# Enter-tainer/oavif

Measured on AMD Instinct MI355X. Metric: ssimulacra2_megapixels_per_sec, higher is better.
Workload: dtype f32; 1 GPU; ssimulacra2 score of one 3840x2160 RGB8 (ref, dist) pair per step per GPU (BASELINE configs[1]); steps rotate over 16 distinct pairs per GPU = 796 MB of frames resident in HBM (> the 256 MiB Infinity Cache); width=3840, height=2160, distinct_pairs_per_gpu=16, parallelism=single gpu, streams_per_gpu=2

## Files before the change

include/ssimu2_hip_internal.h:

```cpp
#ifndef SSIMU2_HIP_INTERNAL_H_
#define SSIMU2_HIP_INTERNAL_H_

#include "ssimu2_hip.h"

#ifdef __cplusplus
extern "C" {
#endif
#if defined(__GNUC__)
#pragma GCC visibility push(default)
#endif

enum { SSIMU2_DEBUG_LIN_REF = 0, SSIMU2_DEBUG_LIN_DIST = 1, SSIMU2_DEBUG_XYB_REF = 2, SSIMU2_DEBUG_REF_BLUR = 3,
       SSIMU2_DEBUG_RG_H = 4, SSIMU2_DEBUG_RG_V = 5 };
int ssimu2_debug_download(ssimu2_ctx* ctx, int what, int scale, uint32_t w, uint32_t h, float* out,
                          uint32_t* out_w, uint32_t* out_h);

int ssimu2_time_device(ssimu2_ctx* ctx, const void* d_ref, const void* d_dist, uint32_t w,
                       uint32_t h, int iters, float* out_ms_total, double* out_score);

enum { SSIMU2_STAGE_PYRAMID = 0, SSIMU2_STAGE_MARCH = 1, SSIMU2_STAGE_FINALIZE = 2 };
int ssimu2_time_stage(ssimu2_ctx* ctx, const void* d_ref, const void* d_dist, uint32_t w, uint32_t h,
                      int stage, int iters, float* out_ms_avg);

int ssimu2_time_march_rotating(ssimu2_ctx* ctx, const void* const* d_refs, const void* const* d_dists,
                               int npairs, uint32_t w, uint32_t h, int iters, float* out_ms_avg);

int ssimu2_measure_read_stream(ssimu2_ctx* ctx, size_t bytes, int iters, double* out_gbps);

int ssimu2_instr_set_segment_rows(ssimu2_ctx* ctx, int rows_scale0, int rows_other_scales);
int ssimu2_instr_cache_reference_blur(ssimu2_ctx* ctx, int enabled);
int ssimu2_instr_set_batch_segment_rows(ssimu2_ctx* ctx, int rows_scale0);
int ssimu2_instr_batch_segment_rows(ssimu2_ctx* ctx, uint32_t w, uint32_t h, int scale, int* out_rows);
int ssimu2_time_blur_stage_rotating(ssimu2_ctx* ctx, const void* const* d_frames, int nframes, uint32_t w,
                                    uint32_t h, int iters, float* out_ms_avg, double* out_bytes_per_launch);
int ssimu2_time_kernels(ssimu2_ctx* ctx, const void* d_ref, const void* const* d_refs, const void* const* d_dists, int n,
                        uint32_t w, uint32_t h, int iters, float* out_ms_avg, int* out_launches, float* out_ms_wall_timed,
                        float* out_ms_wall_plain);
int ssimu2_instr_placed_streams(ssimu2_ctx* ctx, int* out_n);
int ssimu2_instr_rg_stop_after_scale(ssimu2_ctx* ctx, int scale);

#if defined(__GNUC__)
#pragma GCC visibility pop
#endif
#ifdef __cplusplus
}
#endif
#endif
```

oavif_amd/_lib.py:

```python
from __future__ import annotations

import ctypes
import os

_HERE = os.path.dirname(os.path.abspath(__file__))
LIB_PATH = os.environ.get("OAVIF_AMD_LIB") or os.path.join(_HERE, "lib", "liboavif_hip.so")
INSTR_LIB_PATH = os.environ.get("OAVIF_AMD_INSTR_LIB") or os.path.join(_HERE, "lib", "liboavif_hip_instr.so")

OK = 0
ERR_INVALID_ARG = -1
ERR_UNSUPPORTED = -2
ERR_OOM = -3
ERR_HIP = -4
ERR_NO_REFERENCE = -5
ERR_NO_DEVICE = -6

STAGE_PYRAMID, STAGE_MARCH, STAGE_FINALIZE = 0, 1, 2
NUM_SCALES = 6
STATS_PER_SCALE = 18
TQ_MAX_PASS = 12
MAX_BATCH = 4096

BLUR_FIR, BLUR_RECURSIVE, BLUR_RECURSIVE_FMA = 0, 1, 2

# ... 57 lines not shown

    def __init__(self):
        super().__init__()
        self.struct_size = ctypes.sizeof(DeviceInfo)

    def as_dict(self) -> dict:
        return {"device": int(self.device), "arch": self.arch.decode(), "name": self.name.decode(),
                "pci_bus_id": self.pci_bus_id.decode(), "compute_units": int(self.compute_units),
                "lds_bytes_per_cu": int(self.lds_bytes_per_cu), "lds_bytes_per_workgroup": int(self.lds_bytes_per_workgroup),
                "wavefront_size": int(self.wavefront_size), "hbm_bytes": int(self.hbm_bytes),
                "numa_node": int(self.numa_node), "usable": bool(self.usable)}


class TQSpecStats(ctypes.Structure):
    _fields_ = [("waves", ctypes.c_uint32), ("probes_issued", ctypes.c_uint32),
                ("cache_hits", ctypes.c_uint32)]


INSTR_SYMBOLS = ("ssimu2_debug_download", "ssimu2_time_device", "ssimu2_time_stage",
                 "ssimu2_time_march_rotating", "ssimu2_measure_read_stream",
                 "ssimu2_instr_set_segment_rows", "ssimu2_instr_cache_reference_blur",
                 "ssimu2_instr_rg_stop_after_scale", "ssimu2_time_blur_stage_rotating",
                 "ssimu2_instr_placed_streams", "ssimu2_time_kernels",
                 "ssimu2_instr_set_batch_segment_rows", "ssimu2_instr_batch_segment_rows")

TQ_MAX_FANOUT = 16
BATCH_PROBE_FN = ctypes.CFUNCTYPE(ctypes.c_int, ctypes.c_void_p, ctypes.POINTER(ctypes.c_uint32),
                                  ctypes.c_uint32, ctypes.POINTER(ctypes.c_double))
PROBE_FN = ctypes.CFUNCTYPE(ctypes.c_int, ctypes.c_void_p, ctypes.c_uint32,
                            ctypes.POINTER(ctypes.c_double))
CODEC_FN = ctypes.CFUNCTYPE(ctypes.c_int, ctypes.c_void_p, ctypes.c_uint32,
                            ctypes.POINTER(ctypes.c_uint8), ctypes.POINTER(ctypes.c_size_t))

_lib = None
_instr = None


def lib() -> ctypes.CDLL:
    global _lib
    if _lib is None:
        _lib = _load(LIB_PATH, False)
    return _lib


def instr_lib() -> ctypes.CDLL:
    global _instr
    if _instr is None:
# ... 71 lines not shown
        L.ssimu2_score_rgb16.restype = ci
        L.ssimu2_set_reference_rgb16.argtypes = [vp, u16p, u32, u32, u32]
        L.ssimu2_set_reference_rgb16.restype = ci
        L.ssimu2_score_against_reference_rgb16.argtypes = [vp, u16p, u32, f64p]
        L.ssimu2_score_against_reference_rgb16.restype = ci
        L.ssimu2_score_against_reference_strided16.argtypes = [vp, u16p, u32, u32, u32, f64p]
        L.ssimu2_score_against_reference_strided16.restype = ci
    if hasattr(L, "ssimu2_score_batch_rgb8"):
        u8pp = ctypes.POINTER(u8p)
        L.ssimu2_score_batch_rgb8.argtypes = [vp, u8pp, u8pp, u32, u32, u32, f64p]
        L.ssimu2_score_batch_rgb8.restype = ci
        L.ssimu2_score_batch_against_reference.argtypes = [vp, u8pp, u32, f64p]
        L.ssimu2_score_batch_against_reference.restype = ci
        L.ssimu2_score_batch_rgb8_device.argtypes = [vp, vp, vp, ctypes.c_size_t, u32, u32, u32, f64p]
        L.ssimu2_score_batch_rgb8_device.restype = ci
        L.ssimu2_score_batch_against_reference_device.argtypes = [vp, vp, ctypes.c_size_t, u32, f64p]
        L.ssimu2_score_batch_against_reference_device.restype = ci
        L.ssimu2_last_batch_averages.argtypes = [vp, u32, f64p, ctypes.POINTER(ci)]
        L.ssimu2_last_batch_averages.restype = ci
    if instrumented:
        sigs = {
            "ssimu2_instr_set_batch_segment_rows": [vp, ci],
            "ssimu2_instr_batch_segment_rows": [vp, u32, u32, ci, ctypes.POINTER(ci)],
            "ssimu2_measure_read_stream": [vp, ctypes.c_size_t, ci, f64p],
            "ssimu2_debug_download": [vp, ci, ci, u32, u32, ctypes.POINTER(ctypes.c_float),
                                      ctypes.POINTER(u32), ctypes.POINTER(u32)],
            "ssimu2_time_device": [vp, vp, vp, u32, u32, ci, ctypes.POINTER(ctypes.c_float), f64p],
            "ssimu2_time_stage": [vp, vp, vp, u32, u32, ci, ci, ctypes.POINTER(ctypes.c_float)],
            "ssimu2_time_march_rotating": [vp, ctypes.POINTER(vp), ctypes.POINTER(vp), ci, u32, u32, ci,
                                           ctypes.POINTER(ctypes.c_float)],
            "ssimu2_instr_set_segment_rows": [vp, ci, ci],
            "ssimu2_instr_cache_reference_blur": [vp, ci],
            "ssimu2_instr_rg_stop_after_scale": [vp, ci],
            "ssimu2_instr_placed_streams": [vp, ctypes.POINTER(ci)],
            "ssimu2_time_blur_stage_rotating": [vp, ctypes.POINTER(vp), ci, u32, u32, ci,
                                                ctypes.POINTER(ctypes.c_float), f64p],
            "ssimu2_time_kernels": [vp, vp, ctypes.POINTER(vp), ctypes.POINTER(vp), ci, u32, u32, ci, ctypes.POINTER(ctypes.c_float),
                                    ctypes.POINTER(ci), ctypes.POINTER(ctypes.c_float), ctypes.POINTER(ctypes.c_float)],
        }
        for name, argtypes in sigs.items():
            if hasattr(L, name):
                getattr(L, name).argtypes = argtypes
                getattr(L, name).restype = ci
    L.ssimu2_version.argtypes = []
    L.ssimu2_version.restype = ctypes.c_char_p
    L.oavif_tq_default_options.argtypes = [ctypes.POINTER(TQOptions)]
# ... 29 lines not shown
```

oavif_amd/csrc/ssimu2_hip.hip:

```cpp
#include <hip/hip_runtime.h>
#ifdef SSIMU2_INSTRUMENTED_BUILD
#include <hip/hip_ext.h>
#endif

#include <ctype.h>
#include <math.h>
#include <stdint.h>
#include <stdio.h>
#include <stdlib.h>
#include <string.h>
#include <time.h>

#include <future>
#include <mutex>
#include <new>
#include <string>

#include "../../include/ssimu2_hip.h"
#include "ssimu2_kernels.h"
#include "ssimu2_recursive.h"

using namespace ssimu2;

namespace {
// ... 125 lines not shown
    void* d_ref16 = nullptr;
    void* d_dist16 = nullptr;
    void* d_lin0_ref = nullptr;
    void* d_lin0_dist = nullptr;
    size_t cap_ref16 = 0, cap_dist16 = 0, cap_lin0_ref = 0, cap_lin0_dist = 0;
    bool ref_hbd = false;
    void* b_u8_ref = nullptr;
    void* b_u8_dist = nullptr;
    void* b_lin_ref = nullptr;
    void* b_lin_dist = nullptr;
    void* b_part = nullptr;
    size_t cap_b_u8_ref = 0, cap_b_u8_dist = 0, cap_b_lin_ref = 0, cap_b_lin_dist = 0, cap_b_part = 0;
    double* bh_result = nullptr;
    size_t cap_bh_result = 0;
    uint32_t batch_n = 0;

    bool have_ref = false;
    uint32_t ref_w = 0, ref_h = 0;
    bool pending = false;

    hipEvent_t ev0 = nullptr, ev1 = nullptr;
    int seg_rows_override = 0;
    int seg_rows_tail_override = 0;
    int batch_seg_override = 0;
    bool cache_ref_blur = true;
    int rg_dbg_scale = -1;
#ifdef SSIMU2_INSTRUMENTED_BUILD
    uint32_t lin0_ref_w = 0, lin0_ref_h = 0, lin0_dist_w = 0, lin0_dist_h = 0;
#endif

    int fail(int code, const char* what, hipError_t e = hipSuccess) {
        char buf[256];
        if (e != hipSuccess) snprintf(buf, sizeof buf, "%s: %s", what, hipGetErrorString(e));
        else snprintf(buf, sizeof buf, "%s", what);
        err = buf;
        return code;
    }
};

namespace {

#define HIP_TRY(ctx, call)                                                   \
    do {                                                                     \
        hipError_t e_ = (call);                                              \
        if (e_ != hipSuccess) return (ctx)->fail(SSIMU2_ERR_HIP, #call, e_); \
    } while (0)
// ... 230 lines not shown
        hb.in[f] = (const uint8_t*)src[f]->px;
        hb.pitch[f] = src[f]->pitch;
        hb.tab[f] = src[f]->tab;
        hb.maxv[f] = src[f]->maxv;
        hb.lin0[f] = lin0 ? lin0[f] : nullptr;
    }
    return hb;
}

void launch_pyramid16(ssimu2_ctx* c, const Pyramid& p, int nframes, const Src16* const* src, float* const* lin,
                      float* const* lin0) {
    if (p.nscales < 1) return;
    const uint8_t* none[2] = {nullptr, nullptr};
    const PyrBandArgs a = pyramid_args(p, nframes, none, lin);
    const PyrHbdArgs hb = hbd_args(nframes, src, lin0);
    launch(src[0]->ch == 4 ? k_pyramid_bands16<4> : k_pyramid_bands16<3>, dim3(a.bands_x * a.bands_y * nframes),
           dim3(PYR_THREADS), 0, c->stream, a, hb);
}

size_t xyb_off(const Pyramid& p, int s) {
    size_t off = 0;
    for (int k = 0; k < s; ++k) off += (size_t)3 * p.w[k] * p.h[k];
    return off;
}

void build_plans(const ssimu2_ctx* c, const Pyramid& p, const uint8_t* d_ref, const uint8_t* d_dist,
                 bool ref_xyb_cached, MarchPlan* mp, FinalizeArgs* fa, int* total_blocks) {
    memset(mp, 0, sizeof *mp);
    memset(fa, 0, sizeof *fa);
    mp->nscales = fa->nscales = p.nscales;
    size_t poff = 0;
    int blocks = 0;
    for (int s = 0; s < p.nscales; ++s) {
        const int seg = march_seg_rows(c, p, s);
        const int nstrips = (p.w[s] + MW - 1) / MW;
        const int nb = nstrips * ((p.h[s] + seg - 1) / seg);
        blocks += nb;
        mp->blk_end[s] = blocks;
        mp->w[s] = p.w[s];
        mp->h[s] = p.h[s];
        mp->seg[s] = seg;
        mp->nstrips[s] = nstrips;
        mp->nblocks[s] = nb;
        mp->ref[s] = s == 0 ? (const void*)d_ref : (const void*)(c->d_lin_ref + p.lin_off[s]);
        mp->dist[s] = s == 0 ? (const void*)d_dist : (const void*)(c->d_lin_dist + p.lin_off[s]);
        mp->ref_xyb[s] = ref_xyb_cached ? c->d_xyb_ref + xyb_off(p, s) : nullptr;
// ... 181 lines not shown
            if (fma) launch((k_rg_v_emit<true, 3>), dim3(vblocks), dim3(192), 0, c->stream, rp);
            else launch((k_rg_v_emit<false, 3>), dim3(vblocks), dim3(192), 0, c->stream, rp);
        }
    }
    launch(k_finalize, dim3(1), dim3(1024), 0, c->stream, fa, c->h_result);
    HIP_TRY(c, hipGetLastError());
    c->pending = true;
    return SSIMU2_OK;
}

int enqueue_score(ssimu2_ctx* c, const uint8_t* d_ref, const uint8_t* d_dist, uint32_t w, uint32_t h,
                  bool ref_pyramid_ready) {
    const Pyramid p = make_pyramid(w, h);
    const bool recursive = c->blur_mode != SSIMU2_BLUR_FIR;
    note_lin0(c, 0, 0, w, h);
    if (recursive) {
        int rc = rg_check_size(c, w, h);
        if (rc) return rc;
        const bool had_ref = c->have_ref;
        if ((rc = rg_ensure(c, p))) return rc;
        if (ref_pyramid_ready && had_ref && !c->have_ref)
            return c->fail(SSIMU2_ERR_NO_REFERENCE, "recursive blur mode: the cached reference was dropped");
    }
    if (p.nscales > 1 && !recursive) {
        if (ref_pyramid_ready) {
            const uint8_t* frames[1] = {d_dist};
            float* lin[1] = {c->d_lin_dist};
            launch_pyramid(c, p, 1, frames, lin);
        } else {
            const uint8_t* frames[2] = {d_ref, d_dist};
            float* lin[2] = {c->d_lin_ref, c->d_lin_dist};
            launch_pyramid(c, p, 2, frames, lin);
        }
    }
    if (recursive) {
        if (!ref_pyramid_ready) rg_enqueue_reference(c, p, d_ref);
        return rg_enqueue_pass(c, p, d_dist);
    }
    MarchPlan mp;
    FinalizeArgs fa;
    int blocks = 0;
    build_plans(c, p, d_ref, d_dist, ref_pyramid_ready && c->d_xyb_ref != nullptr, &mp, &fa, &blocks);
    if (blocks > 0) {
        if (mp.ref_s11[0])
            launch(k_march_refblur, dim3(blocks), dim3(MARCH_THREADS), 0, c->stream, mp);
        else
            launch(k_march, dim3(blocks), dim3(MARCH_THREADS), 0, c->stream, mp);
    }
    launch(k_finalize, dim3(1), dim3(1024), 0, c->stream, fa, c->h_result);
    HIP_TRY(c, hipGetLastError());
    c->pending = true;
    return SSIMU2_OK;
}

int enqueue_score16(ssimu2_ctx* c, const Src16* ref, const Src16& dist, uint32_t w, uint32_t h) {
    const Pyramid p = make_pyramid(w, h);
    if (c->blur_mode != SSIMU2_BLUR_FIR) {
        int rc = rg_check_size(c, w, h);
        if (rc) return rc;
        const bool had_ref = c->have_ref;
        if ((rc = rg_ensure(c, p))) return rc;
        if (!ref && had_ref && !c->have_ref)
            return c->fail(SSIMU2_ERR_NO_REFERENCE, "recursive blur mode: the cached reference was dropped");
        if (ref) rg_enqueue_reference(c, p, nullptr, ref);
        return rg_enqueue_pass(c, p, nullptr, &dist);
    }
// ... 1123 lines not shown
```

oavif_amd/csrc/ssimu2_instrument.hip:

```cpp
#define SSIMU2_INSTRUMENTED_BUILD 1
#include "ssimu2_hip.hip"

#include "../../include/ssimu2_hip_internal.h"

namespace ssimu2 {

__global__ __launch_bounds__(256) void k_read_stream(const uint4* __restrict__ src, size_t n16,
                                                     uint32_t* __restrict__ sink) {
    const size_t chunk = (n16 + gridDim.x - 1) / gridDim.x;
    const size_t lo = (size_t)blockIdx.x * chunk;
    const size_t hi = lo + chunk < n16 ? lo + chunk : n16;
    size_t i = lo + threadIdx.x;
    uint4 acc = make_uint4(0, 0, 0, 0);
    for (; i + 768 < hi; i += 1024) {
        const uint4 a = src[i], b = src[i + 256], c = src[i + 512], d = src[i + 768];
        acc.x ^= a.x ^ b.x ^ c.x ^ d.x;
        acc.y ^= a.y ^ b.y ^ c.y ^ d.y;
        acc.z ^= a.z ^ b.z ^ c.z ^ d.z;
        acc.w ^= a.w ^ b.w ^ c.w ^ d.w;
    }
    for (; i < hi; i += 256) {
        const uint4 a = src[i];
        acc.x ^= a.x; acc.y ^= a.y; acc.z ^= a.z; acc.w ^= a.w;
    }
// ... 7 lines not shown

int ssimu2_instr_set_segment_rows(ssimu2_ctx* c, int rows_scale0, int rows_other_scales) {
    if (!c) return SSIMU2_ERR_INVALID_ARG;
    if ((rows_scale0 != 0 && (rows_scale0 < 8 || rows_scale0 > 160)) ||
        (rows_other_scales != 0 && (rows_other_scales < 8 || rows_other_scales > 160)))
        return c->fail(SSIMU2_ERR_INVALID_ARG, "segment rows must be 0 (default rule) or 8..160");
    HIP_TRY(c, hipSetDevice(c->device));
    HIP_TRY(c, hipStreamSynchronize(c->stream));
    c->seg_rows_override = rows_scale0;
    c->seg_rows_tail_override = rows_other_scales;
    free_buffers(c);
    c->have_ref = false;
    return SSIMU2_OK;
}

int ssimu2_instr_set_batch_segment_rows(ssimu2_ctx* c, int rows_scale0) {
    if (!c) return SSIMU2_ERR_INVALID_ARG;
    if (rows_scale0 != 0 && rows_scale0 != -1 && (rows_scale0 < 8 || rows_scale0 > 160))
        return c->fail(SSIMU2_ERR_INVALID_ARG, "batch segment rows must be 0 (the rule), -1 (the single-score rule) or 8..160");
    HIP_TRY(c, hipSetDevice(c->device));
    HIP_TRY(c, hipStreamSynchronize(c->stream));
    c->batch_seg_override = rows_scale0;
    return SSIMU2_OK;
}

int ssimu2_instr_batch_segment_rows(ssimu2_ctx* c, uint32_t w, uint32_t h, int scale, int* out_rows) {
    if (!c || !out_rows || scale < 0 || scale >= kNumScales || w == 0 || h == 0) return SSIMU2_ERR_INVALID_ARG;
    *out_rows = batch_seg_rows(c, make_pyramid(w, h), scale);
    return SSIMU2_OK;
}

int ssimu2_instr_placed_streams(ssimu2_ctx* c, int* out_n) {
    if (!c || !out_n) return SSIMU2_ERR_INVALID_ARG;
    *out_n = pool_size(c->device);
    return SSIMU2_OK;
}

int ssimu2_instr_rg_stop_after_scale(ssimu2_ctx* c, int scale) {
    if (!c) return SSIMU2_ERR_INVALID_ARG;
    c->rg_dbg_scale = scale < 0 || scale >= kNumScales ? -1 : scale;
    return SSIMU2_OK;
}

int ssimu2_instr_cache_reference_blur(ssimu2_ctx* c, int enabled) {
    if (!c) return SSIMU2_ERR_INVALID_ARG;
    c->cache_ref_blur = enabled != 0;
// ... 357 lines not shown
```

oavif_amd/csrc/ssimu2_kernels.h:

```cpp
#pragma once

#include <hip/hip_runtime.h>
#include <stdint.h>

#include "../../include/ssimu2_hip.h"

namespace ssimu2 {

constexpr int kNumScales = SSIMU2_NUM_SCALES;
constexpr int kStats = SSIMU2_STATS_PER_SCALE;

constexpr float kC2 = 0.0009f;
constexpr float kM00 = 0.30f, kM01 = 0.622f, kM02 = 0.078f;
constexpr float kM10 = 0.23f, kM11 = 0.692f, kM12 = 0.078f;
constexpr float kM20 = 0.24342268924547819f, kM21 = 0.20476744424496821f,
                kM22 = 0.55180986650955360f;
constexpr float kOpsinBias = 0.0037930732552754493f;

struct DevConst {
    float lut[256];
    float taps[5];
    float cbrt_bias;
    float rg_n2[3];
    float rg_d1[3];
// ... 377 lines not shown
    __shared__ float s_lut[256];
    __shared__ float s_tiles[PYR_BAND_LDS_FLOATS];
    if (threadIdx.x < 256) s_lut[threadIdx.x] = c_k.lut[threadIdx.x];
    __syncthreads();
    pyramid_band<false>(a, (int)blockIdx.x, s_lut, s_tiles);
}

struct PyrBatchArgs {
    PyrBandArgs a;
    size_t in_stride;
    size_t out_stride;
};
__global__ __launch_bounds__(PYR_THREADS) void k_pyramid_bands_batch(PyrBatchArgs b) {
    __shared__ float s_lut[256];
    __shared__ float s_tiles[PYR_BAND_LDS_FLOATS];
    if (threadIdx.x < 256) s_lut[threadIdx.x] = c_k.lut[threadIdx.x];
    __syncthreads();
    const int per_item = b.a.bands_x * b.a.bands_y * b.a.nframes;
    const int item = (int)blockIdx.x / per_item;
    pyramid_band<false, 0, true>(b.a, (int)blockIdx.x - item * per_item, s_lut, s_tiles, nullptr, (size_t)item * b.in_stride,
                        (size_t)item * b.out_stride);
}

__global__ __launch_bounds__(PYR_THREADS) void k_pyramid_bands_xyb(PyrBandArgs a) {
    __shared__ float s_lut[256];
    __shared__ float s_tiles[PYR_BAND_LDS_FLOATS];
    if (threadIdx.x < 256) s_lut[threadIdx.x] = c_k.lut[threadIdx.x];
    if (blockIdx.x == 0 && threadIdx.x < 4 && a.zero4) a.zero4[threadIdx.x] = 0u;
    __syncthreads();
    pyramid_band<true>(a, (int)blockIdx.x, s_lut, s_tiles);
}

template <int CH>
__global__ __launch_bounds__(PYR_THREADS) void k_pyramid_bands16(PyrBandArgs a, PyrHbdArgs hb) {
    __shared__ float s_tiles[PYR_BAND_LDS_FLOATS];
    pyramid_band<false, CH>(a, (int)blockIdx.x, nullptr, s_tiles, &hb);
}

template <int CH>
__global__ __launch_bounds__(PYR_THREADS) void k_pyramid_bands_xyb16(PyrBandArgs a, PyrHbdArgs hb) {
    __shared__ float s_tiles[PYR_BAND_LDS_FLOATS];
    if (blockIdx.x == 0 && threadIdx.x < 4 && a.zero4) a.zero4[threadIdx.x] = 0u;
    __syncthreads();
    pyramid_band<true, CH>(a, (int)blockIdx.x, nullptr, s_tiles, &hb);
}

// ... 85 lines not shown
template <bool U8>
__device__ __forceinline__ void march_load(uint32_t (&raw)[3], MarchCursor& c, int row) {
    const uint8_t* p = c.base + (size_t)(uint32_t)row * (uint32_t)c.pitch;
    asm volatile("" : "+v"(c.off));
    const uint32_t off = c.off;
    if (U8) {
        uint32_t d;
        __builtin_memcpy(&d, p + off, 4);
        raw[0] = d;
    } else {
        raw[0] = *(const uint32_t*)(p + off);
        raw[1] = *(const uint32_t*)((p + c.plane) + off);
        raw[2] = *(const uint32_t*)((p + 2 * c.plane) + off);
    }
}

__device__ __forceinline__ void march_lut(const float* lut, uint32_t d, uint32_t shift, float (&lin)[3]) {
    d >>= shift;
    lin[0] = lut[d & 255u];
    lin[1] = lut[(d >> 8) & 255u];
    lin[2] = lut[(d >> 16) & 255u];
}

template <bool U8, int MODE, bool LIN0 = false, bool BATCH = false>
__device__ __forceinline__ void march_convert_rows(f2 (*ring)[3][MRW], const float* lut,
                                                   const MarchPlan& plan, int sc, int w, int h, int x0,
                                                   int y0, int steps, int ngroups, int col, size_t off0 = 0,
                                                   size_t off1 = 0) {
    constexpr bool CACHED = MODE == MARCH_REFBLUR || MODE == MARCH_EMIT;
    constexpr bool TWO = MODE != MARCH_EMIT;
    constexpr bool LUT0 = U8 && !CACHED;
    const int gx = x0 - RAD + col;
    const bool col_ok = gx >= 0 && gx < w;
    const bool all_cols = x0 - RAD >= 0 && x0 - RAD + MRW <= w;
    const int gxc = min(max(gx, 0), w - 1);
    MarchCursor c0 = CACHED ? march_cursor<false>(plan.ref_xyb[sc], w, h, gxc)
                            : march_cursor<U8>(plan.ref[sc], w, h, gxc);
    MarchCursor c1 = march_cursor<U8>(plan.dist[sc], w, h, gxc);
    if constexpr (BATCH) {
        if (!CACHED) c0.base += off0;
        c1.base += off1;
    }
    int load_row = y0 - RAD;
    constexpr int NG = 2;
    constexpr int QD = NG * GROUP;
    uint32_t raw0[QD][3], raw1[QD][3];
    float lin0[3] = {0.f, 0.f, 0.f}, lin1[3] = {0.f, 0.f, 0.f};
#define MARCH_LOAD(J)                                                      \
    {                                                                      \
        const int lrow_ = min(max(load_row, 0), h - 1);       \
        if (CACHED) march_load<false>(raw0[J], c0, lrow_);                 \
        else march_load<U8>(raw0[J], c0, lrow_);                           \
        if (TWO) march_load<U8>(raw1[J], c1, lrow_);                       \
        ++load_row;                                                        \
    }
#define MARCH_LUT(J)                                                             \
    if (U8) {                                                                    \
        if (LUT0) march_lut(lut, raw0[J][0], c0.shift, lin0);                    \
        if (TWO) march_lut(lut, raw1[J][0], c1.shift, lin1);                     \
    }
#define MARCH_PUT(J, R)                                                                        \
    {                                                                                          \
           \
                              \
        const bool rok_ = (unsigned)(y0 - RAD + (R)) < (unsigned)h;                            \
        float a_[3] = {0.f, 0.f, 0.f}, b_[3] = {0.f, 0.f, 0.f};                                \
        float m0_[3], m1_[3];                                                                  \
        if (!CACHED) {                                                                         \
            if (U8) opsin_mix(lin0[0], lin0[1], lin0[2], m0_);                                 \
            else opsin_mix(__uint_as_float(raw0[J][0]), __uint_as_float(raw0[J][1]),           \
                           __uint_as_float(raw0[J][2]), m0_);                                  \
        }                                                                                      \
        if (TWO) {                                                                             \
            if (U8) opsin_mix(lin1[0], lin1[1], lin1[2], m1_);                                 \
            else opsin_mix(__uint_as_float(raw1[J][0]), __uint_as_float(raw1[J][1]),           \
                           __uint_as_float(raw1[J][2]), m1_);                                  \
        }                                                                                      \
        if (U8) {                                                                              \
            __builtin_amdgcn_sched_barrier(0);                                                 \
            MARCH_LUT((J + 1) % QD)                                                            \
            __builtin_amdgcn_sched_barrier(0);                                                 \
        }                                                                                      \
        if (CACHED) {                                                                          \
            _Pragma("unroll") for (int c_ = 0; c_ < 3; ++c_) a_[c_] = __uint_as_float(raw0[J][c_]); \
        } else {                                                                               \
            mixed_to_xyb_pos(m0_, a_);                                                         \
        }                                                                                      \
        if (TWO) mixed_to_xyb_pos(m1_, b_);                                                    \
        if (!(all_cols && rok_)) {     \
            asm volatile("; zero padding");                                                    \
            const bool keep_ = col_ok && rok_;                                                 \
            _Pragma("unroll") for (int c_ = 0; c_ < 3; ++c_) {                                 \
                a_[c_] = keep_ ? a_[c_] : 0.0f;                                                \
                b_[c_] = keep_ ? b_[c_] : 0.0f;                                                \
            }                                                                                  \
        }                                                                                      \
        _Pragma("unroll") for (int c_ = 0; c_ < 3; ++c_)                                       \
            ring[(R) & (RING - 1)][c_][col] = f2{a_[c_], b_[c_]};                              \
    }
#pragma unroll
// ... 144 lines not shown
    acc[2] += art;
    acc[3] += a2 * a2;
    acc[4] += det;
    acc[5] += t2 * t2;
}

__device__ __forceinline__ int march_tile_of_block(int b, int first, int end) {
    const int x = b & 7;
    int before = 0;
#pragma unroll
    for (int r = 0; r < 8; ++r) {
        const int n_r = (end + 7 - r) / 8 - (first + 7 - r) / 8;
        before += r < x ? n_r : 0;
    }
    return before + (b >> 3) - ((first + 7 - x) >> 3);
}

struct MarchItem {
    int sc, tile;
    size_t off_ref, off_dist;
    size_t off_part;
};

template <int MODE, bool LIN0 = false, bool BATCH = false>
__device__ __forceinline__ void march_body(const MarchPlan& plan, const MapCoef* coef = nullptr,
                                           const MarchItem* it = nullptr) {
    __shared__ __attribute__((aligned(16))) f2 s_ring[RING][3][MRW];
    __shared__ float s_lut[256];
    __shared__ double s_part[6][6];
    const int tid = threadIdx.x, lane = tid & 63;
    const int wave = __builtin_amdgcn_readfirstlane(tid >> 6);

    int sc = 0, first = 0;
#pragma unroll
    for (int s = 0; s < kNumScales - 1; ++s)
        if (!BATCH && s + 1 < plan.nscales && (int)blockIdx.x >= plan.blk_end[s]) {
            sc = s + 1;
            first = plan.blk_end[s];
        }
    if constexpr (BATCH) sc = it->sc;
    const int blk = BATCH ? it->tile : march_tile_of_block((int)blockIdx.x, first, plan.blk_end[sc]);
    const int w = plan.w[sc], h = plan.h[sc], seg_rows = plan.seg[sc];
    const int nstrips = plan.nstrips[sc];
    const int by = blk / nstrips, bx = blk - by * nstrips;
    const bool u8 = !LIN0 && sc == 0;
    const int x0 = bx * MW;
    const int y0 = by * seg_rows;
    const int rows_out = min(seg_rows, h - y0);
    const int steps = rows_out + 2 * RAD;
    if (u8) {
        for (int i = tid; i < 256; i += MARCH_THREADS) s_lut[i] = c_k.lut[i];
    }
    __syncthreads();

    const float w0 = c_k.taps[0], w1 = c_k.taps[1], w2 = c_k.taps[2], w3 = c_k.taps[3],
                w4 = c_k.taps[4];
    const bool is_conv = wave < CONV_WAVES;
    float acc[6] = {0.f, 0.f, 0.f, 0.f, 0.f, 0.f};
    const int hw = wave - CONV_WAVES;
// ... 3 lines not shown
    const bool ok = x0 + o < w;
    MarchRefBlur rb;
    rb.pitch = w;
    rb.rows_left = rows_out;
    rb.active = hv_active;
#pragma unroll
    for (int k = 0; k < 9; ++k) rb.ps11[k] = 0.f;
    float mc[6] = {0.f, 0.f, 0.f, 0.f, 0.f, 0.f};
    if (MODE == MARCH_MAP) {
        const int cc = max(ch, 0);
        mc[0] = coef->c[sc][cc * 2];
        mc[1] = coef->c[sc][cc * 2 + 1];
#pragma unroll
        for (int k = 0; k < 4; ++k) mc[2 + k] = coef->c[sc][6 + cc * 4 + k];
    }
    {
        const size_t at = ((size_t)max(ch, 0) * h + y0) * (size_t)w + (size_t)min(x0 + o, w - 1);
        rb.s11 = MODE == MARCH_PAIR ? nullptr : plan.ref_s11[sc] + at;
    }

    const int ngroups = (steps + GROUP - 1) / GROUP;
    if (is_conv) {
        const int col = (wave << 6) + lane;
        if constexpr (BATCH) {
            if (u8) march_convert_rows<true, MODE, LIN0, true>(s_ring, s_lut, plan, sc, w, h, x0, y0, steps, ngroups, col, it->off_ref, it->off_dist);
            else march_convert_rows<false, MODE, LIN0, true>(s_ring, s_lut, plan, sc, w, h, x0, y0, steps, ngroups, col, it->off_ref, it->off_dist);
        } else {
            if (u8) march_convert_rows<true, MODE, LIN0>(s_ring, s_lut, plan, sc, w, h, x0, y0, steps, ngroups, col);
            else march_convert_rows<false, MODE, LIN0>(s_ring, s_lut, plan, sc, w, h, x0, y0, steps, ngroups, col);
        }
    } else {
        float win[5][9];
        const lds_vu64* rp = (const lds_vu64*)&s_ring[0][ch][o];
        const bool edge = x0 + MW > w;
        __syncthreads();
#define MARCH_STEP(P)                                                                          \
    {                                                                                          \
        const int t = t0 + P;                                                                  \
        if (t < steps) march_h<P, MODE>(rp, win, t, w0, w1, w2, w3, w4);                       \
        if ((P % GROUP) == GROUP - 1 && t - (GROUP - 1) < steps) __syncthreads();              \
        if (t < steps) march_v<P, MODE>(rp, win, acc, t, ok, edge, w0, w1, w2, w3, w4, rb, mc);    \
    }
#pragma unroll 1
        for (int t0 = 0; t0 < steps; t0 += 9) {
            MARCH_STEP(0)
            MARCH_STEP(1)
            MARCH_STEP(2)
// ... 56 lines not shown
        tile = v - item * nb;
    }
    item = __builtin_amdgcn_readfirstlane(item);
    tile = __builtin_amdgcn_readfirstlane(tile);
    MarchItem it;
    it.sc = sc;
    it.tile = tile;
    it.off_ref = (size_t)item * (sc == 0 ? bp.ref_stride0 : bp.ref_stride);
    it.off_dist = (size_t)item * (sc == 0 ? bp.dist_stride0 : bp.dist_stride);
    it.off_part = (size_t)item * bp.part_stride;
    march_body<MODE, false, true>(bp.item, nullptr, &it);
}

__global__ __launch_bounds__(MARCH_THREADS, 6) void k_march(MarchPlan plan) {
    march_body<MARCH_PAIR>(plan);
}

__global__ __launch_bounds__(MARCH_THREADS, 6) void k_march_refblur(MarchPlan plan) {
    march_body<MARCH_REFBLUR>(plan);
}

__global__ __launch_bounds__(MARCH_THREADS, 6) void k_ref_blur(MarchPlan plan) {
    march_body<MARCH_EMIT>(plan);
}

__global__ __launch_bounds__(MARCH_THREADS, 6) void k_march_lin(MarchPlan plan) {
    march_body<MARCH_PAIR, true>(plan);
}

__global__ __launch_bounds__(MARCH_THREADS, 6) void k_march_refblur_lin(MarchPlan plan) {
    march_body<MARCH_REFBLUR, true>(plan);
}

__global__ __launch_bounds__(MARCH_THREADS, 6) void k_march_batch(MarchBatchPlan bp) {
    march_batch_body<MARCH_PAIR, false>(bp);
}

__global__ __launch_bounds__(MARCH_THREADS, 6) void k_march_refblur_batch(MarchBatchPlan bp) {
    march_batch_body<MARCH_REFBLUR, true>(bp);
}

__global__ __launch_bounds__(MARCH_THREADS, 6) void k_march_map(MarchPlan plan, MapCoef coef) {
    march_body<MARCH_MAP>(plan, &coef);
}

struct MapComposeArgs {
// ... 165 lines not shown
```

oavif_amd/scorer.py:

```python
from __future__ import annotations

import ctypes

import numpy as np

from . import _lib


class Ssimu2Error(RuntimeError):
    def __init__(self, code: int, msg: str):
        super().__init__(f"ssimu2 error {code}: {msg}")
        self.code = code


def _u8p(a: np.ndarray):
    return a.ctypes.data_as(ctypes.POINTER(ctypes.c_uint8))


def _f32p(a: np.ndarray):
    return a.ctypes.data_as(ctypes.POINTER(ctypes.c_float))


def _check_rgb8(a, name: str) -> np.ndarray:
    a = np.ascontiguousarray(a, dtype=np.uint8)
# ... 370 lines not shown
    def last_batch_averages(self, item: int):
        avg = np.zeros(_lib.NUM_SCALES * _lib.STATS_PER_SCALE, np.float64)
        ns = ctypes.c_int()
        rc = self._L.ssimu2_last_batch_averages(self._ctx, int(item), avg.ctypes.data_as(ctypes.POINTER(ctypes.c_double)),
                                                ctypes.byref(ns))
        if rc != 0:
            self._raise(rc)
        return avg.reshape(_lib.NUM_SCALES, _lib.STATS_PER_SCALE), ns.value

    def set_batch_segment_rows(self, rows_scale0: int) -> None:
        self._need_instr()
        rc = self._L.ssimu2_instr_set_batch_segment_rows(self._ctx, int(rows_scale0))
        if rc != 0:
            self._raise(rc)

    def batch_segment_rows(self, w: int, h: int, scale: int) -> int:
        self._need_instr()
        rows = ctypes.c_int()
        rc = self._L.ssimu2_instr_batch_segment_rows(self._ctx, int(w), int(h), int(scale), ctypes.byref(rows))
        if rc != 0:
            self._raise(rc)
        return int(rows.value)

    def _need_instr(self):
        if not self.instrumented:
            raise RuntimeError("this hook needs Ssimu2(..., instrumented=True) (liboavif_hip_instr.so)")

    def time_device(self, d_ref: int, d_dist: int, w: int, h: int, iters: int):
        self._need_instr()
        ms = ctypes.c_float()
        out = ctypes.c_double()
        rc = self._L.ssimu2_time_device(self._ctx, ctypes.c_void_p(d_ref), ctypes.c_void_p(d_dist),
                                        w, h, iters, ctypes.byref(ms), ctypes.byref(out))
        if rc != 0:
            self._raise(rc)
        return ms.value, out.value

    def time_stage(self, d_ref: int, d_dist: int, w: int, h: int, stage: int, iters: int) -> float:
        self._need_instr()
        ms = ctypes.c_float()
        rc = self._L.ssimu2_time_stage(self._ctx, ctypes.c_void_p(d_ref), ctypes.c_void_p(d_dist),
                                       w, h, stage, iters, ctypes.byref(ms))
        if rc != 0:
            self._raise(rc)
        return ms.value

# ... 47 lines not shown
        arr = ctypes.c_void_p * n
        ms = ctypes.c_float()
        rc = self._L.ssimu2_time_march_rotating(self._ctx, arr(*d_refs), arr(*d_dists), n, w, h, iters,
                                                ctypes.byref(ms))
        if rc != 0:
            self._raise(rc)
        return ms.value

    def time_blur_stage_rotating(self, d_frames, w: int, h: int, iters: int):
        self._need_instr()
        n = len(d_frames)
        arr = ctypes.c_void_p * n
        ms, nbytes = ctypes.c_float(), ctypes.c_double()
        rc = self._L.ssimu2_time_blur_stage_rotating(self._ctx, arr(*d_frames), n, w, h, iters,
                                                     ctypes.byref(ms), ctypes.byref(nbytes))
        if rc != 0:
            self._raise(rc)
        return ms.value, nbytes.value

    KERNEL_NAMES = {(False, True): ("pyramid", "march_refblur", "finalize"), (False, False): ("pyramid", "march", "finalize"),
                    (True, True): ("convert", "h", "v", "finalize"),
                    (True, False): ("ref_convert", "ref_h", "ref_v_emit", "convert", "h", "v", "finalize")}

    def time_kernels(self, w: int, h: int, d_dists, iters: int, d_ref: int | None = None, d_refs=None, recursive: bool = False):
        self._need_instr()
        n = len(d_dists)
        arr = ctypes.c_void_p * n
        ms = (ctypes.c_float * 8)()
        nl = ctypes.c_int()
        wt, wp = ctypes.c_float(), ctypes.c_float()
        rc = self._L.ssimu2_time_kernels(self._ctx, ctypes.c_void_p(d_ref or 0), arr(*d_refs) if d_refs is not None else None,
                                         arr(*d_dists), n, w, h, iters, ms, ctypes.byref(nl), ctypes.byref(wt), ctypes.byref(wp))
        if rc != 0:
            self._raise(rc)
        if d_refs is None:
            self._ref_shape = (h, w, 3)
        names = self.KERNEL_NAMES[(bool(recursive), d_refs is None)]
        if nl.value != len(names):
            names = tuple(f"launch{k}" for k in range(nl.value))
        return dict(zip(names, (float(ms[k]) for k in range(nl.value)))), float(wt.value), float(wp.value)

    def set_segment_rows(self, rows_scale0: int, rows_other_scales: int) -> None:
        self._need_instr()
        rc = self._L.ssimu2_instr_set_segment_rows(self._ctx, rows_scale0, rows_other_scales)
        if rc != 0:
            self._raise(rc)

    def cache_reference_blur(self, enabled: bool) -> None:
        self._need_instr()
        rc = self._L.ssimu2_instr_cache_reference_blur(self._ctx, 1 if enabled else 0)
        if rc != 0:
            self._raise(rc)

    def last_averages(self):
        avg = np.zeros(_lib.NUM_SCALES * _lib.STATS_PER_SCALE, np.float64)
        ns = ctypes.c_int()
        rc = self._L.ssimu2_last_averages(self._ctx,
                                          avg.ctypes.data_as(ctypes.POINTER(ctypes.c_double)),
                                          ctypes.byref(ns))
        if rc != 0:
# ... 19 lines not shown
```

Before: 55200 MP/s.

## Fold pyramid levels 1-2 into the scale-0 march kernel for large pairs

For pair scoring at sizes of at least 2560x1440, the separate pyramid kernel is skipped. The scale-0 march kernel now writes the 2x and 4x downsampled linear planes from its in-register LUT values, using DPP lane shifts to average neighbouring columns. A small LDS kernel then builds levels 3-5 from level 2, and a third launch runs the march for the remaining scales. This avoids reading both full-resolution RGB8 frames a second time to build the pyramid. In exchange it adds scattered stores and extra registers inside the march kernel, and splits the march into separate launches that run one after another.

```diff
diff --git a/include/ssimu2_hip_internal.h b/include/ssimu2_hip_internal.h
--- a/include/ssimu2_hip_internal.h
+++ b/include/ssimu2_hip_internal.h
@@ -31,6 +31,8 @@
 int ssimu2_instr_cache_reference_blur(ssimu2_ctx* ctx, int enabled);
 int ssimu2_instr_set_batch_segment_rows(ssimu2_ctx* ctx, int rows_scale0);
 int ssimu2_instr_batch_segment_rows(ssimu2_ctx* ctx, uint32_t w, uint32_t h, int scale, int* out_rows);
+int ssimu2_instr_set_pair_pyramid_path(ssimu2_ctx* ctx, int mode);
+int ssimu2_instr_pair_pyramid_folded(uint32_t w, uint32_t h);
 int ssimu2_time_blur_stage_rotating(ssimu2_ctx* ctx, const void* const* d_frames, int nframes, uint32_t w,
                                     uint32_t h, int iters, float* out_ms_avg, double* out_bytes_per_launch);
 int ssimu2_time_kernels(ssimu2_ctx* ctx, const void* d_ref, const void* const* d_refs, const void* const* d_dists, int n,
diff --git a/oavif_amd/_lib.py b/oavif_amd/_lib.py
--- a/oavif_amd/_lib.py
+++ b/oavif_amd/_lib.py
@@ -103,7 +103,8 @@
                  "ssimu2_instr_set_segment_rows", "ssimu2_instr_cache_reference_blur",
                  "ssimu2_instr_rg_stop_after_scale", "ssimu2_time_blur_stage_rotating",
                  "ssimu2_instr_placed_streams", "ssimu2_time_kernels",
-                 "ssimu2_instr_set_batch_segment_rows", "ssimu2_instr_batch_segment_rows")
+                 "ssimu2_instr_set_batch_segment_rows", "ssimu2_instr_batch_segment_rows",
+                 "ssimu2_instr_set_pair_pyramid_path", "ssimu2_instr_pair_pyramid_folded")
 
 TQ_MAX_FANOUT = 16
 BATCH_PROBE_FN = ctypes.CFUNCTYPE(ctypes.c_int, ctypes.c_void_p, ctypes.POINTER(ctypes.c_uint32),
@@ -221,6 +222,8 @@
         sigs = {
             "ssimu2_instr_set_batch_segment_rows": [vp, ci],
             "ssimu2_instr_batch_segment_rows": [vp, u32, u32, ci, ctypes.POINTER(ci)],
+            "ssimu2_instr_set_pair_pyramid_path": [vp, ci],
+            "ssimu2_instr_pair_pyramid_folded": [u32, u32],
             "ssimu2_measure_read_stream": [vp, ctypes.c_size_t, ci, f64p],
             "ssimu2_debug_download": [vp, ci, ci, u32, u32, ctypes.POINTER(ctypes.c_float),
                                       ctypes.POINTER(u32), ctypes.POINTER(u32)],
diff --git a/oavif_amd/csrc/ssimu2_hip.hip b/oavif_amd/csrc/ssimu2_hip.hip
--- a/oavif_amd/csrc/ssimu2_hip.hip
+++ b/oavif_amd/csrc/ssimu2_hip.hip
@@ -171,6 +171,7 @@
     hipEvent_t ev0 = nullptr, ev1 = nullptr;
     int seg_rows_override = 0;
     int seg_rows_tail_override = 0;
+    int pair_pyramid_override = 0;
     int batch_seg_override = 0;
     bool cache_ref_blur = true;
     int rg_dbg_scale = -1;
@@ -447,6 +448,31 @@
     size_t off = 0;
     for (int k = 0; k < s; ++k) off += (size_t)3 * p.w[k] * p.h[k];
     return off;
+}
+
+bool pair_pyramid_can_fold(const Pyramid& p) {
+    return p.nscales == kNumScales && p.w[0] % 4 == 0 && p.h[0] % 4 == 0;
+}
+constexpr uint64_t kFoldMinPixels = (uint64_t)2560 * 1440;
+bool pair_pyramid_folded(uint32_t w, uint32_t h) {
+    return (uint64_t)w * h >= kFoldMinPixels && pair_pyramid_can_fold(make_pyramid(w, h));
+}
+
+PyrTailArgs pyramid_tail_args(const ssimu2_ctx* c, const Pyramid& p) {
+    PyrTailArgs a{};
+    a.nlevels = p.nscales - 3;
+    for (int l = 2; l < p.nscales; ++l) {
+        a.w[l - 2] = p.w[l];
+        a.h[l - 2] = p.h[l];
+    }
+    float* lin[2] = {c->d_lin_ref, c->d_lin_dist};
+    for (int f = 0; f < 2; ++f) {
+        a.in[f] = lin[f] + p.lin_off[2];
+        for (int l = 0; l < a.nlevels; ++l) a.out[f][l] = lin[f] + p.lin_off[3 + l];
+    }
+    a.bands_x = (p.w[2] + PYT_TX - 1) / PYT_TX;
+    a.bands_y = (p.h[2] + 7) / 8;
+    return a;
 }
 
 void build_plans(const ssimu2_ctx* c, const Pyramid& p, const uint8_t* d_ref, const uint8_t* d_dist,
@@ -674,7 +700,9 @@
         if (ref_pyramid_ready && had_ref && !c->have_ref)
             return c->fail(SSIMU2_ERR_NO_REFERENCE, "recursive blur mode: the cached reference was dropped");
     }
-    if (p.nscales > 1 && !recursive) {
+    const bool fold = !recursive && !ref_pyramid_ready && pair_pyramid_can_fold(p) &&
+                      (c->pair_pyramid_override ? c->pair_pyramid_override > 0 : pair_pyramid_folded(w, h));
+    if (p.nscales > 1 && !recursive && !fold) {
         if (ref_pyramid_ready) {
             const uint8_t* frames[1] = {d_dist};
             float* lin[1] = {c->d_lin_dist};
@@ -693,7 +721,20 @@
     FinalizeArgs fa;
     int blocks = 0;
     build_plans(c, p, d_ref, d_dist, ref_pyramid_ready && c->d_xyb_ref != nullptr, &mp, &fa, &blocks);
-    if (blocks > 0) {
+    if (fold) {
+        MarchPyrOut po{};
+        po.l1[0] = c->d_lin_ref + p.lin_off[1];
+        po.l1[1] = c->d_lin_dist + p.lin_off[1];
+        po.l2[0] = c->d_lin_ref + p.lin_off[2];
+        po.l2[1] = c->d_lin_dist + p.lin_off[2];
+        po.w1 = p.w[1], po.h1 = p.h[1], po.w2 = p.w[2], po.h2 = p.h[2];
+        const int blocks0 = mp.blk_end[0];
+        launch(k_march_pyr, dim3(blocks0), dim3(MARCH_THREADS), 0, c->stream, mp, po);
+        const PyrTailArgs ta = pyramid_tail_args(c, p);
+        launch(k_pyramid_tail, dim3(ta.bands_x * ta.bands_y * 2), dim3(PYT_THREADS), 0, c->stream, ta);
+        for (int s = 0; s < p.nscales; ++s) mp.blk_end[s] -= blocks0;
+        launch(k_march, dim3(blocks - blocks0), dim3(MARCH_THREADS), 0, c->stream, mp);
+    } else if (blocks > 0) {
         if (mp.ref_s11[0])
             launch(k_march_refblur, dim3(blocks), dim3(MARCH_THREADS), 0, c->stream, mp);
         else
diff --git a/oavif_amd/csrc/ssimu2_instrument.hip b/oavif_amd/csrc/ssimu2_instrument.hip
--- a/oavif_amd/csrc/ssimu2_instrument.hip
+++ b/oavif_amd/csrc/ssimu2_instrument.hip
@@ -53,6 +53,17 @@
     HIP_TRY(c, hipStreamSynchronize(c->stream));
     c->batch_seg_override = rows_scale0;
     return SSIMU2_OK;
+}
+
+int ssimu2_instr_set_pair_pyramid_path(ssimu2_ctx* c, int mode) {
+    if (!c) return SSIMU2_ERR_INVALID_ARG;
+    if (mode < -1 || mode > 1) return c->fail(SSIMU2_ERR_INVALID_ARG, "pair pyramid path must be 0 (the size rule), 1 (folded) or -1 (classic)");
+    c->pair_pyramid_override = mode;
+    return SSIMU2_OK;
+}
+
+int ssimu2_instr_pair_pyramid_folded(uint32_t w, uint32_t h) {
+    return w != 0 && h != 0 && pair_pyramid_folded(w, h) ? 1 : 0;
 }
 
 int ssimu2_instr_batch_segment_rows(ssimu2_ctx* c, uint32_t w, uint32_t h, int scale, int* out_rows) {
diff --git a/oavif_amd/csrc/ssimu2_kernels.h b/oavif_amd/csrc/ssimu2_kernels.h
--- a/oavif_amd/csrc/ssimu2_kernels.h
+++ b/oavif_amd/csrc/ssimu2_kernels.h
@@ -423,6 +423,51 @@
                         (size_t)item * b.out_stride);
 }
 
+struct PyrTailArgs {
+    const float* in[2];
+    float* out[2][3];
+    int w[4], h[4];
+    int nlevels;
+    int bands_x, bands_y;
+};
+constexpr int PYT_TX = 32;
+constexpr int PYT_THREADS = 8 * PYT_TX;
+__global__ __launch_bounds__(PYT_THREADS) void k_pyramid_tail(PyrTailArgs a) {
+    constexpr int TX = PYT_TX;
+    __shared__ float s2[3 * 8 * TX];
+    __shared__ float s3[3 * 4 * (TX / 2)];
+    __shared__ float s4[3 * 2 * (TX / 4)];
+    const int t = threadIdx.x;
+    const int per_frame = a.bands_x * a.bands_y;
+    const int f = (int)blockIdx.x / per_frame;
+    const int r = (int)blockIdx.x - f * per_frame;
+    const int by = r / a.bands_x, bx = r - by * a.bands_x;
+    const int tx = t % TX, ty = t / TX;
+    {
+        const int w2 = a.w[0], h2 = a.h[0];
+        const int ox = bx * TX + tx, oy = by * 8 + ty;
+        const size_t n2 = (size_t)w2 * h2;
+        const float* in = a.in[f];
+#pragma unroll
+        for (int c = 0; c < 3; ++c)
+            s2[(c * 8 + ty) * TX + tx] = ox < w2 && oy < h2 ? in[c * n2 + (size_t)oy * w2 + ox] : 0.f;
+    }
+    __syncthreads();
+    if (t < 4 * (TX / 2))
+        pyr_lds_level<false>(s2, TX, 8, a.w[0], a.h[0], s3, TX / 2, 4, a.out[f][0], a.w[1], a.h[1], a.w[1], bx * (TX / 2),
+                             by * 4, t % (TX / 2), t / (TX / 2));
+    if (a.nlevels < 2) return;
+    __syncthreads();
+    if (t < 2 * (TX / 4))
+        pyr_lds_level<false>(s3, TX / 2, 4, a.w[1], a.h[1], s4, TX / 4, 2, a.out[f][1], a.w[2], a.h[2], a.w[2], bx * (TX / 4),
+                             by * 2, t % (TX / 4), t / (TX / 4));
+    if (a.nlevels < 3) return;
+    __syncthreads();
+    if (t < TX / 8)
+        pyr_lds_level<false>(s4, TX / 4, 2, a.w[2], a.h[2], nullptr, 0, 0, a.out[f][2], a.w[3], a.h[3], a.w[3], bx * (TX / 8), by,
+                             t, 0);
+}
+
 __global__ __launch_bounds__(PYR_THREADS) void k_pyramid_bands_xyb(PyrBandArgs a) {
     __shared__ float s_lut[256];
     __shared__ float s_tiles[PYR_BAND_LDS_FLOATS];
@@ -554,11 +599,80 @@
     lin[2] = lut[(d >> 16) & 255u];
 }
 
-template <bool U8, int MODE, bool LIN0 = false, bool BATCH = false>
+struct MarchPyrOut {
+    float* l1[2];
+    float* l2[2];
+    int w1, h1, w2, h2;
+};
+
+struct MarchPyr {
+    float s0[3], s1[3];
+    float t0[3], t1[3];
+    uint32_t off1, off2;
+    bool st1, st2;
+};
+
+template <int N>
+__device__ __forceinline__ float march_dpp_right(float v) {
+    return __uint_as_float((uint32_t)__builtin_amdgcn_update_dpp(0, (int)__float_as_uint(v), 0x100 + N, 0xf, 0xf, true));
+}
+
+__device__ __forceinline__ void march_pyr_store(float* base, int pitch, int rows, int row, uint32_t& off,
+                                                const float (&v)[3]) {
+    uint8_t* p = (uint8_t*)base + (size_t)(uint32_t)row * (uint32_t)pitch * 4;
+    const size_t plane = (size_t)pitch * rows * 4;
+    asm volatile("" : "+v"(off));
+    const uint32_t o = off;
+    *(float*)(p + o) = v[0];
+    *(float*)((p + plane) + o) = v[1];
+    *(float*)((p + 2 * plane) + o) = v[2];
+}
+
+__device__ __forceinline__ void march_pyr_row(MarchPyr& q, const MarchPyrOut& po, int yr, int y0, int rows_out,
+                                              const float (&lin0)[3], const float (&lin1)[3]) {
+    if (!(yr & 1)) {
+#pragma unroll
+        for (int c = 0; c < 3; ++c) {
+            q.s0[c] = lin0[c] + march_dpp_right<1>(lin0[c]);
+            q.s1[c] = lin1[c] + march_dpp_right<1>(lin1[c]);
+        }
+        return;
+    }
+    float a[3], b[3];
+#pragma unroll
+    for (int c = 0; c < 3; ++c) {
+        a[c] = ((q.s0[c] + lin0[c]) + march_dpp_right<1>(lin0[c])) * 0.25f;
+        b[c] = ((q.s1[c] + lin1[c]) + march_dpp_right<1>(lin1[c])) * 0.25f;
+    }
+    if ((unsigned)(yr - 1 - y0) < (unsigned)rows_out && q.st1) {
+        march_pyr_store(po.l1[0], po.w1, po.h1, (yr - 1) >> 1, q.off1, a);
+        march_pyr_store(po.l1[1], po.w1, po.h1, (yr - 1) >> 1, q.off1, b);
+    }
+    if (!(yr & 2)) {
+#pragma unroll
+        for (int c = 0; c < 3; ++c) {
+            q.t0[c] = a[c] + march_dpp_right<2>(a[c]);
+            q.t1[c] = b[c] + march_dpp_right<2>(b[c]);
+        }
+        return;
+    }
+#pragma unroll
+    for (int c = 0; c < 3; ++c) {
+        a[c] = ((q.t0[c] + a[c]) + march_dpp_right<2>(a[c])) * 0.25f;
+        b[c] = ((q.t1[c] + b[c]) + march_dpp_right<2>(b[c])) * 0.25f;
+    }
+    if ((unsigned)(yr - 3 - y0) < (unsigned)rows_out && q.st2) {
+        march_pyr_store(po.l2[0], po.w2, po.h2, (yr - 3) >> 2, q.off2, a);
+        march_pyr_store(po.l2[1], po.w2, po.h2, (yr - 3) >> 2, q.off2, b);
+    }
+}
+
+template <bool U8, int MODE, bool LIN0 = false, bool BATCH = false, bool PYR = false>
 __device__ __forceinline__ void march_convert_rows(f2 (*ring)[3][MRW], const float* lut,
                                                    const MarchPlan& plan, int sc, int w, int h, int x0,
                                                    int y0, int steps, int ngroups, int col, size_t off0 = 0,
-                                                   size_t off1 = 0) {
+                                                   size_t off1 = 0, const MarchPyrOut* po = nullptr) {
+    static_assert(!PYR || (U8 && MODE == MARCH_PAIR && !BATCH), "the pyramid comes from the LUT values of both frames");
     constexpr bool CACHED = MODE == MARCH_REFBLUR || MODE == MARCH_EMIT;
     constexpr bool TWO = MODE != MARCH_EMIT;
     constexpr bool LUT0 = U8 && !CACHED;
@@ -578,6 +692,16 @@
     constexpr int QD = NG * GROUP;
     uint32_t raw0[QD][3], raw1[QD][3];
     float lin0[3] = {0.f, 0.f, 0.f}, lin1[3] = {0.f, 0.f, 0.f};
+    MarchPyr pyr{};
+    if constexpr (PYR) {
+        const int oc = col - RAD;
+        const int ox1 = (x0 + oc) >> 1;
+        const bool own = oc >= 0 && oc < MW;
+        pyr.st1 = own && !(oc & 1) && ox1 < po->w1;
+        pyr.st2 = own && !(oc & 3) && (ox1 >> 1) < po->w2;
+        pyr.off1 = (uint32_t)max(ox1, 0) * 4u;
+        pyr.off2 = (uint32_t)max(ox1 >> 1, 0) * 4u;
+    }
 #define MARCH_LOAD(J)                                                      \
     {                                                                      \
         const int lrow_ = min(max(load_row, 0), h - 1);       \
@@ -608,6 +732,7 @@
             else opsin_mix(__uint_as_float(raw1[J][0]), __uint_as_float(raw1[J][1]),           \
                            __uint_as_float(raw1[J][2]), m1_);                                  \
         }                                                                                      \
+        if constexpr (PYR) march_pyr_row(pyr, *po, y0 - RAD + (R), y0, steps - 2 * RAD, lin0, lin1); \
         if (U8) {                                                                              \
             __builtin_amdgcn_sched_barrier(0);                                                 \
             MARCH_LUT((J + 1) % QD)                                                            \
@@ -798,9 +923,9 @@
     size_t off_part;
 };
 
-template <int MODE, bool LIN0 = false, bool BATCH = false>
+template <int MODE, bool LIN0 = false, bool BATCH = false, bool PYR = false>
 __device__ __forceinline__ void march_body(const MarchPlan& plan, const MapCoef* coef = nullptr,
-                                           const MarchItem* it = nullptr) {
+                                           const MarchItem* it = nullptr, const MarchPyrOut* po = nullptr) {
     __shared__ __attribute__((aligned(16))) f2 s_ring[RING][3][MRW];
     __shared__ float s_lut[256];
     __shared__ double s_part[6][6];
@@ -810,7 +935,7 @@
     int sc = 0, first = 0;
 #pragma unroll
     for (int s = 0; s < kNumScales - 1; ++s)
-        if (!BATCH && s + 1 < plan.nscales && (int)blockIdx.x >= plan.blk_end[s]) {
+        if (!BATCH && !PYR && s + 1 < plan.nscales && (int)blockIdx.x >= plan.blk_end[s]) {
             sc = s + 1;
             first = plan.blk_end[s];
         }
@@ -860,7 +985,9 @@
     const int ngroups = (steps + GROUP - 1) / GROUP;
     if (is_conv) {
         const int col = (wave << 6) + lane;
-        if constexpr (BATCH) {
+        if constexpr (PYR) {
+            march_convert_rows<true, MODE, false, false, true>(s_ring, s_lut, plan, sc, w, h, x0, y0, steps, ngroups, col, 0, 0, po);
+        } else if constexpr (BATCH) {
             if (u8) march_convert_rows<true, MODE, LIN0, true>(s_ring, s_lut, plan, sc, w, h, x0, y0, steps, ngroups, col, it->off_ref, it->off_dist);
             else march_convert_rows<false, MODE, LIN0, true>(s_ring, s_lut, plan, sc, w, h, x0, y0, steps, ngroups, col, it->off_ref, it->off_dist);
         } else {
@@ -963,6 +1090,10 @@
 
 __global__ __launch_bounds__(MARCH_THREADS, 6) void k_ref_blur(MarchPlan plan) {
     march_body<MARCH_EMIT>(plan);
+}
+
+__global__ __launch_bounds__(MARCH_THREADS, 6) void k_march_pyr(MarchPlan plan, MarchPyrOut po) {
+    march_body<MARCH_PAIR, false, false, true>(plan, nullptr, nullptr, &po);
 }
 
 __global__ __launch_bounds__(MARCH_THREADS, 6) void k_march_lin(MarchPlan plan) {
diff --git a/oavif_amd/scorer.py b/oavif_amd/scorer.py
--- a/oavif_amd/scorer.py
+++ b/oavif_amd/scorer.py
@@ -416,6 +416,16 @@
             self._raise(rc)
         return int(rows.value)
 
+    def set_pair_pyramid_path(self, mode: int) -> None:
+        self._need_instr()
+        rc = self._L.ssimu2_instr_set_pair_pyramid_path(self._ctx, int(mode))
+        if rc != 0:
+            self._raise(rc)
+
+    def pair_pyramid_folded(self, w: int, h: int) -> bool:
+        self._need_instr()
+        return bool(self._L.ssimu2_instr_pair_pyramid_folded(int(w), int(h)))
+
     def _need_instr(self):
         if not self.instrumented:
             raise RuntimeError("this hook needs Ssimu2(..., instrumented=True) (liboavif_hip_instr.so)")
@@ -509,6 +519,8 @@
                     (True, True): ("convert", "h", "v", "finalize"),
                     (True, False): ("ref_convert", "ref_h", "ref_v_emit", "convert", "h", "v", "finalize")}
 
+    KERNEL_NAMES_FOLDED = ("march0", "pyramid_tail", "march", "finalize")
+
     def time_kernels(self, w: int, h: int, d_dists, iters: int, d_ref: int | None = None, d_refs=None, recursive: bool = False):
         self._need_instr()
         n = len(d_dists)
@@ -523,6 +535,8 @@
         if d_refs is None:
             self._ref_shape = (h, w, 3)
         names = self.KERNEL_NAMES[(bool(recursive), d_refs is None)]
+        if not recursive and d_refs is not None and nl.value == len(self.KERNEL_NAMES_FOLDED):
+            names = self.KERNEL_NAMES_FOLDED
         if nl.value != len(names):
             names = tuple(f"launch{k}" for k in range(nl.value))
         return dict(zip(names, (float(ms[k]) for k in range(nl.value)))), float(wt.value), float(wp.value)
```

Result: slower. 53850 MP/s (-2.4%).
